# OpenRobotLab/EmbodiedScan

Hardware: AMD Instinct MI355X
Metric: scans/sec (train step) mv-3ddet, 20x(480x640) RGB-D views (higher is better)
Workload: dtype bf16; 1 GPU; mv-3ddet ResNet-50(w16) + MinkResNet34 + FCAF3DHeadRotMat, 20 views 480x640, 100k points/scan, bf16 matrix cores with f32 accumulate / f32 master weights, full train step incl. H2D of the batch and AdamW; views=20, parallelism=dp1, h2d=157 MB per step as ONE copy from a pinned slab on a copy stream, double-buffered

## Files before the change

### embodiedscan_amd/csrc/rowops.hip

```cpp
#include "common.h"
#include "../../include/es_hip.h"

int ES_OPT_NORM_CHUNK = 0;
static int norm_chunk_rows(int max_rows) {
  if (ES_OPT_NORM_CHUNK > 0) return ES_OPT_NORM_CHUNK;
  return max_rows <= (1 << 17) ? 128 : (max_rows <= (1 << 18) ? 256 : 512);
}
#define FCH 16
#define FST 64

struct Segs { int n; int off[ES_MAX_SEG + 1]; };
__device__ inline int seg_of(const Segs& s, int row) {
  int g = 0;
  for (int i = 1; i < s.n; ++i) g += (row >= s.off[i]);
  return g;
}
static Segs make_segs(const int* seg_off, int nseg) {
  Segs s;
  s.n = nseg;
  for (int i = 0; i <= nseg; ++i) s.off[i] = seg_off[i];
  return s;
}
static int max_seg_rows(const Segs& s) {
  int m = 0;
// ... 120 lines not shown
                                                     const float* __restrict__ res, int ldr, int act,
                                                     float* __restrict__ y, int ldy, unsigned short* __restrict__ yh) {
  const int C4 = C >> 2;
  const size_t tot = (size_t)n * C4, stride = (size_t)gridDim.x * blockDim.x;
  for (size_t e0 = (size_t)blockIdx.x * blockDim.x + threadIdx.x; e0 < tot; e0 += 2 * stride) {
    size_t e1 = e0 + stride;
    bool v1 = e1 < tot;
    int r0 = (int)(e0 / C4), c0 = (int)(e0 - (size_t)r0 * C4) * 4;
    int r1 = v1 ? (int)(e1 / C4) : r0, c1 = v1 ? (int)(e1 - (size_t)r1 * C4) * 4 : c0;
    float4 x0 = *(const float4*)(x + (size_t)r0 * ldx + c0), x1 = *(const float4*)(x + (size_t)r1 * ldx + c1);
    float4 q0 = make_float4(0, 0, 0, 0), q1 = q0;
    if (res) { q0 = *(const float4*)(res + (size_t)r0 * ldr + c0); q1 = *(const float4*)(res + (size_t)r1 * ldr + c1); }
#define NA_ONE(xv, qv, r, c)                                                                                   \
    {                                                                                                          \
      int sg = seg_of(segs, r);                                                                                \
      float4 m = *(const float4*)(mean + sg * C + c), is = *(const float4*)(invstd + sg * C + c);             \
      float4 ww = *(const float4*)(w + c), bb = *(const float4*)(b + c);                                       \
      float z0 = (xv.x - m.x) * is.x * ww.x + bb.x, z1 = (xv.y - m.y) * is.y * ww.y + bb.y;                    \
      float z2 = (xv.z - m.z) * is.z * ww.z + bb.z, z3 = (xv.w - m.w) * is.w * ww.w + bb.w;                    \
      if (res) { z0 += qv.x; z1 += qv.y; z2 += qv.z; z3 += qv.w; }                                             \
      z0 = act_fwd(z0, act); z1 = act_fwd(z1, act); z2 = act_fwd(z2, act); z3 = act_fwd(z3, act);             \
      *(float4*)(y + (size_t)r * ldy + c) = make_float4(z0, z1, z2, z3);                                       \
      if (yh) *(uint2*)(yh + (size_t)r * C + c) = make_uint2(es_pack_bf16(z0, z1), es_pack_bf16(z2, z3));      \
    }
    NA_ONE(x0, q0, r0, c0)
    if (v1) NA_ONE(x1, q1, r1, c1)
#undef NA_ONE
  }
}

int ES_OPT_ELECT_SAFE = 0;
int ES_OPT_NORM_CB_ROWS = 4096;
int ES_OPT_NORM_CB_BWD = 1;
#define NCB_TY 128
#define NCB_WAVES 8
__device__ inline void cb_reduce4(double v[4], double (*sm)[4][4]) {
  const int lane = threadIdx.x & 63, wv = threadIdx.x >> 6, tx = threadIdx.x & 3;
#pragma unroll
  for (int i = 0; i < 4; ++i) {
#pragma unroll
    for (int o = 4; o < 64; o <<= 1) v[i] += __shfl_xor(v[i], o, 64);
  }
  __syncthreads();
  if ((lane >> 2) == 0) {
#pragma unroll
    for (int i = 0; i < 4; ++i) sm[wv][tx][i] = v[i];
  }
  __syncthreads();
#pragma unroll
  for (int i = 0; i < 4; ++i) {
    double tot = 0;
#pragma unroll
    for (int w = 0; w < NCB_WAVES; ++w) tot += sm[w][tx][i];
    v[i] = tot;
  }
}
__global__ __launch_bounds__(512) void k_norm_fwd_cb(const float* __restrict__ x, int ldx, int n, int C, float eps,
                                                      const float* __restrict__ w, const float* __restrict__ b,
                                                      const float* __restrict__ res, int ldr, int act, float* running_mean,
                                                      float* running_var, float momentum, float* __restrict__ mean,
                                                      float* __restrict__ invstd, float* __restrict__ y, int ldy,
                                                      unsigned short* __restrict__ yh) {
  __shared__ double sm[NCB_WAVES][4][4];
  const int tx = threadIdx.x & 3, ty = threadIdx.x >> 2, c = blockIdx.x * 16 + tx * 4;
  const float4 k = *(const float4*)(x + c);
  float4 s = make_float4(0, 0, 0, 0), q = make_float4(0, 0, 0, 0);
  for (int rb = ty; rb < n; rb += 4 * NCB_TY) {
    float4 v[4];
#pragma unroll
    for (int u = 0; u < 4; ++u) {
      const int r = rb + u * NCB_TY;
      const float4 t = *(const float4*)(x + (size_t)(r < n ? r : rb) * ldx + c);
      v[u].x = r < n ? t.x : k.x; v[u].y = r < n ? t.y : k.y;
      v[u].z = r < n ? t.z : k.z; v[u].w = r < n ? t.w : k.w;
    }
#pragma unroll
    for (int u = 0; u < 4; ++u) {
      float dx = v[u].x - k.x, dy = v[u].y - k.y, dz = v[u].z - k.z, dw = v[u].w - k.w;
      s.x += dx; s.y += dy; s.z += dz; s.w += dw;
      q.x += dx * dx; q.y += dy * dy; q.z += dz * dz; q.w += dw * dw;
    }
  }
  double a[4] = {s.x, s.y, s.z, s.w}, bq[4] = {q.x, q.y, q.z, q.w};
  cb_reduce4(a, sm);
  cb_reduce4(bq, sm);
  const double inv_n = 1.0 / (double)n;
  const float kk[4] = {k.x, k.y, k.z, k.w};
  float m4[4], is4[4];
#pragma unroll
  for (int i = 0; i < 4; ++i) {
    double ms = a[i] * inv_n, var = bq[i] * inv_n - ms * ms;
    if (var < 0) var = 0;
    m4[i] = (float)((double)kk[i] + ms);
    is4[i] = (float)(1.0 / sqrt(var + (double)eps));
    if (ty == 0) {
      mean[c + i] = m4[i];
      invstd[c + i] = is4[i];
      if (running_mean && n > 1) {
        running_mean[c + i] = (1.f - momentum) * running_mean[c + i] + momentum * m4[i];
        running_var[c + i] = (1.f - momentum) * running_var[c + i] + momentum * (float)(var * n / (n - 1));
      }
    }
  }
  const float4 ww = *(const float4*)(w + c), bb = *(const float4*)(b + c);
  for (int rb = ty; rb < n; rb += 4 * NCB_TY) {
    float4 v[4], qv[4];
#pragma unroll
    for (int u = 0; u < 4; ++u) {
      int r = rb + u * NCB_TY;
      int rc = r < n ? r : rb;
      v[u] = *(const float4*)(x + (size_t)rc * ldx + c);
      if (res) qv[u] = *(const float4*)(res + (size_t)rc * ldr + c);
    }
#pragma unroll
    for (int u = 0; u < 4; ++u) {
      int r = rb + u * NCB_TY;
      if (r >= n) continue;
      float z0 = (v[u].x - m4[0]) * is4[0] * ww.x + bb.x, z1 = (v[u].y - m4[1]) * is4[1] * ww.y + bb.y;
      float z2 = (v[u].z - m4[2]) * is4[2] * ww.z + bb.z, z3 = (v[u].w - m4[3]) * is4[3] * ww.w + bb.w;
      if (res) { z0 += qv[u].x; z1 += qv[u].y; z2 += qv[u].z; z3 += qv[u].w; }
      z0 = act_fwd(z0, act); z1 = act_fwd(z1, act); z2 = act_fwd(z2, act); z3 = act_fwd(z3, act);
      *(float4*)(y + (size_t)r * ldy + c) = make_float4(z0, z1, z2, z3);
      if (yh) *(uint2*)(yh + (size_t)r * C + c) = make_uint2(es_pack_bf16(z0, z1), es_pack_bf16(z2, z3));
    }
  }
}
static bool norm_cb_ok(int n, int C, int nseg) {
  return ES_OPT_NORM_CB_ROWS > 0 && nseg == 1 && n >= 1 && n <= ES_OPT_NORM_CB_ROWS && (C & 15) == 0;
}

extern "C" int es_norm_fwd(const float* x, int ldx, int n, int C, const int* seg_off, int nseg, float eps,
                           const float* weight, const float* bias, const float* res, int ldr, int act,
                           float* running_mean, float* running_var, float momentum, float* mean, float* invstd,
                           float* workspace, float* y, int ldy, void* y_bf16, void* stream) {
  hipStream_t st = (hipStream_t)stream;
  if (n <= 0 || nseg > ES_MAX_SEG) return nseg > ES_MAX_SEG ? -3 : 0;
  Segs s = make_segs(seg_off, nseg);
  const bool vec0 = ((C & 3) == 0) && ((ldx & 3) == 0) && ((ldy & 3) == 0) && (!res || (ldr & 3) == 0) &&
                    (((((uintptr_t)x) | ((uintptr_t)y) | ((uintptr_t)res) | ((uintptr_t)weight) | ((uintptr_t)bias) |
                       ((uintptr_t)mean) | ((uintptr_t)invstd)) & 15) == 0);
  if (vec0 && norm_cb_ok(n, C, nseg) && seg_off[0] == 0 && seg_off[1] == n) {
    hipLaunchKernelGGL(k_norm_fwd_cb, dim3(C / 16), dim3(4 * NCB_TY), 0, st, x, ldx, n, C, eps, weight, bias, res, ldr, act,
                       running_mean, running_var, momentum, mean, invstd, y, ldy, (unsigned short*)y_bf16);
    ES_CHECK_LAUNCH();
    return 0;
  }
  const int NCH = norm_chunk_rows(max_seg_rows(s));
  int nchunk = es_cdiv(max_seg_rows(s), NCH);
  if (nchunk < 1) nchunk = 1;
  hipLaunchKernelGGL(k_norm_stats, dim3(nchunk, nseg), dim3(256), 0, st, x, ldx, C, s, nchunk, NCH,
                     workspace);
  hipLaunchKernelGGL(k_norm_finalize, dim3(es_cdiv(C, FCH), nseg), dim3(FCH * FST), 0, st, workspace, C, s, nchunk, NCH, eps,
                     mean, invstd, running_mean, running_var, momentum);
  const bool vec = ((C & 3) == 0) && ((ldx & 3) == 0) && ((ldy & 3) == 0) && (!res || (ldr & 3) == 0) &&
                   (((((uintptr_t)x) | ((uintptr_t)y) | ((uintptr_t)res) | ((uintptr_t)weight) | ((uintptr_t)bias) |
                      ((uintptr_t)mean) | ((uintptr_t)invstd)) & 15) == 0);
  if (vec) {
    int g = es_cdiv((long long)n * (C >> 2), 512);
    if (g > 8192) g = 8192;
    hipLaunchKernelGGL(k_norm_apply4, dim3(g < 1 ? 1 : g), dim3(256), 0, st, x, ldx, n, C, s, mean, invstd, weight, bias,
                       res, ldr, act, y, ldy, (unsigned short*)y_bf16);
  } else {
    int g = es_cdiv((long long)n * C, 256);
    if (g > 4096) g = 4096;
    hipLaunchKernelGGL(k_norm_apply, dim3(g), dim3(256), 0, st, x, ldx, n, C, s, mean, invstd, weight, bias, res,
                       ldr, act, y, ldy);
    if (y_bf16) return es_cast_rows_bf16(y, ldy, n, C, y_bf16, stream);
  }
  ES_CHECK_LAUNCH();
  return 0;
}
extern "C" size_t es_norm_workspace_floats(int n, int C, const int* seg_off, int nseg) {
  int m = 0;
  for (int i = 0; i < nseg; ++i) m = max(m, seg_off[i + 1] - seg_off[i]);
  int nchunk = es_cdiv(m, norm_chunk_rows(m));
  if (nchunk < 1) nchunk = 1;
// ... 147 lines not shown
                                                         const float* __restrict__ sum_dzx, float* __restrict__ dx,
                                                         int ldo, int accumulate, unsigned short* __restrict__ dxh) {
  const int C4 = C >> 2;
  const size_t tot = (size_t)n * C4, stride = (size_t)gridDim.x * blockDim.x;
  for (size_t e0 = (size_t)blockIdx.x * blockDim.x + threadIdx.x; e0 < tot; e0 += 2 * stride) {
    size_t e1 = e0 + stride;
    bool v1 = e1 < tot;
    int r0 = (int)(e0 / C4), c0 = (int)(e0 - (size_t)r0 * C4) * 4;
    int r1 = v1 ? (int)(e1 / C4) : r0, c1 = v1 ? (int)(e1 - (size_t)r1 * C4) * 4 : c0;
    float4 x0 = *(const float4*)(x + (size_t)r0 * ldx + c0), x1 = *(const float4*)(x + (size_t)r1 * ldx + c1);
    float4 g0 = *(const float4*)(dz + (size_t)r0 * ldd + c0), g1 = *(const float4*)(dz + (size_t)r1 * ldd + c1);
    float4 o0 = make_float4(0, 0, 0, 0), o1 = o0;
    if (accumulate) { o0 = *(const float4*)(dx + (size_t)r0 * ldo + c0); o1 = *(const float4*)(dx + (size_t)r1 * ldo + c1); }
#define NB_ELT(xe, ge, oe, me, ie, we, se, qe) \
    { float xh = ((xe) - (me)) * (ie); float gg = (we) * (ie) * ((ge) - (se) * inv_n - xh * (qe) * inv_n); oe = accumulate ? ((oe) + gg) : gg; }
#define NB_ONE(xv, gv, ov, r, c)                                                                               \
    {                                                                                                          \
      int sg = seg_of(segs, r);                                                                                \
      float inv_n = 1.f / (float)(segs.off[sg + 1] - segs.off[sg]);                                            \
      float4 m = *(const float4*)(mean + sg * C + c), is = *(const float4*)(invstd + sg * C + c);             \
      float4 ww = *(const float4*)(w + c), sd = *(const float4*)(sum_dz + sg * C + c);                         \
      float4 sq = *(const float4*)(sum_dzx + sg * C + c);                                                      \
      NB_ELT(xv.x, gv.x, ov.x, m.x, is.x, ww.x, sd.x, sq.x) NB_ELT(xv.y, gv.y, ov.y, m.y, is.y, ww.y, sd.y, sq.y) \
      NB_ELT(xv.z, gv.z, ov.z, m.z, is.z, ww.z, sd.z, sq.z) NB_ELT(xv.w, gv.w, ov.w, m.w, is.w, ww.w, sd.w, sq.w) \
      *(float4*)(dx + (size_t)r * ldo + c) = ov;                                                               \
      if (dxh) *(uint2*)(dxh + (size_t)r * C + c) = make_uint2(es_pack_bf16(ov.x, ov.y), es_pack_bf16(ov.z, ov.w)); \
    }
    NB_ONE(x0, g0, o0, r0, c0)
    if (v1) NB_ONE(x1, g1, o1, r1, c1)
#undef NB_ONE
#undef NB_ELT
  }
}
__global__ __launch_bounds__(512) void k_norm_bwd_cb(float* __restrict__ dy, int ldd, const float* __restrict__ y, int ldy,
                                                      const float* __restrict__ x, int ldx, int n, int C,
                                                      const float* __restrict__ mean, const float* __restrict__ invstd,
                                                      const float* __restrict__ w, int act, float* dweight, float* dbias,
                                                      float* __restrict__ dx, int ldo, int accumulate,
                                                      unsigned short* __restrict__ dxh) {
  __shared__ double sm[NCB_WAVES][4][4];
  const int tx = threadIdx.x & 3, ty = threadIdx.x >> 2, c = blockIdx.x * 16 + tx * 4;
  const float4 m = *(const float4*)(mean + c), is = *(const float4*)(invstd + c);
  float4 s = make_float4(0, 0, 0, 0), q = make_float4(0, 0, 0, 0);
  for (int rb = ty; rb < n; rb += 4 * NCB_TY) {
    float4 g[4], yv[4], xv[4];
#pragma unroll
    for (int u = 0; u < 4; ++u) {
      int r = rb + u * NCB_TY;
      int rc = r < n ? r : rb;
      g[u] = *(const float4*)(dy + (size_t)rc * ldd + c);
      if (act) yv[u] = *(const float4*)(y + (size_t)rc * ldy + c);
      xv[u] = *(const float4*)(x + (size_t)rc * ldx + c);
    }
#pragma unroll
    for (int u = 0; u < 4; ++u) {
      int r = rb + u * NCB_TY;
      if (r >= n) continue;
      float4 gg = g[u];
      if (act) {
        float4 yy = yv[u];
        if (act == 1) {
          gg.x = yy.x > 0.f ? gg.x : 0.f; gg.y = yy.y > 0.f ? gg.y : 0.f;
          gg.z = yy.z > 0.f ? gg.z : 0.f; gg.w = yy.w > 0.f ? gg.w : 0.f;
        } else {
          gg.x = yy.x > 0.f ? gg.x : gg.x * (yy.x + 1.f); gg.y = yy.y > 0.f ? gg.y : gg.y * (yy.y + 1.f);
          gg.z = yy.z > 0.f ? gg.z : gg.z * (yy.z + 1.f); gg.w = yy.w > 0.f ? gg.w : gg.w * (yy.w + 1.f);
        }
        *(float4*)(dy + (size_t)r * ldd + c) = gg;
      }
      float4 xx = xv[u];
      s.x += gg.x; s.y += gg.y; s.z += gg.z; s.w += gg.w;
      q.x += gg.x * ((xx.x - m.x) * is.x); q.y += gg.y * ((xx.y - m.y) * is.y);
      q.z += gg.z * ((xx.z - m.z) * is.z); q.w += gg.w * ((xx.w - m.w) * is.w);
    }
  }
  double a[4] = {s.x, s.y, s.z, s.w}, bq[4] = {q.x, q.y, q.z, q.w};
  cb_reduce4(a, sm);
  cb_reduce4(bq, sm);
  if (ty == 0) {
#pragma unroll
    for (int i = 0; i < 4; ++i) {
      if (dweight) dweight[c + i] += (float)bq[i];
      if (dbias) dbias[c + i] += (float)a[i];
    }
  }
  const float sd[4] = {(float)a[0], (float)a[1], (float)a[2], (float)a[3]};
  const float sq[4] = {(float)bq[0], (float)bq[1], (float)bq[2], (float)bq[3]};
  const float4 ww = *(const float4*)(w + c);
  const float inv_n = 1.f / (float)n;
  for (int rb = ty; rb < n; rb += 4 * NCB_TY) {
    float4 g[4], xv[4], ov[4];
#pragma unroll
    for (int u = 0; u < 4; ++u) {
      int r = rb + u * NCB_TY;
      int rc = r < n ? r : rb;
      g[u] = *(const float4*)(dy + (size_t)rc * ldd + c);
      xv[u] = *(const float4*)(x + (size_t)rc * ldx + c);
      ov[u] = accumulate ? *(const float4*)(dx + (size_t)rc * ldo + c) : make_float4(0, 0, 0, 0);
    }
#pragma unroll
    for (int u = 0; u < 4; ++u) {
      int r = rb + u * NCB_TY;
      if (r >= n) continue;
#define NCB_ELT(xe, ge, oe, me, ie, we, se, qe) \
      { float xh = ((xe) - (me)) * (ie); float gg = (we) * (ie) * ((ge) - (se) * inv_n - xh * (qe) * inv_n); oe = accumulate ? ((oe) + gg) : gg; }
      NCB_ELT(xv[u].x, g[u].x, ov[u].x, m.x, is.x, ww.x, sd[0], sq[0]) NCB_ELT(xv[u].y, g[u].y, ov[u].y, m.y, is.y, ww.y, sd[1], sq[1])
      NCB_ELT(xv[u].z, g[u].z, ov[u].z, m.z, is.z, ww.z, sd[2], sq[2]) NCB_ELT(xv[u].w, g[u].w, ov[u].w, m.w, is.w, ww.w, sd[3], sq[3])
#undef NCB_ELT
      *(float4*)(dx + (size_t)r * ldo + c) = ov[u];
      if (dxh) *(uint2*)(dxh + (size_t)r * C + c) = make_uint2(es_pack_bf16(ov[u].x, ov[u].y), es_pack_bf16(ov[u].z, ov[u].w));
    }
  }
}
extern "C" int es_norm_bwd(float* dy, int ldd, const float* y, int ldy, const float* x, int ldx, int n, int C,
                           const int* seg_off, int nseg, const float* mean, const float* invstd,
                           const float* weight, int act, float* dweight, float* dbias, float* workspace, float* dx,
                           int ldo, int accumulate, void* dx_bf16, void* stream) {
  hipStream_t st = (hipStream_t)stream;
  if (n <= 0 || nseg > ES_MAX_SEG) return nseg > ES_MAX_SEG ? -3 : 0;
  Segs s = make_segs(seg_off, nseg);
  const int NCH = norm_chunk_rows(max_seg_rows(s));
  int nchunk = es_cdiv(max_seg_rows(s), NCH);
  if (nchunk < 1) nchunk = 1;
  {
    const bool vec0 = ((C & 3) == 0) && ((ldx & 3) == 0) && ((ldd & 3) == 0) && ((ldo & 3) == 0) && ((ldy & 3) == 0) &&
                      (((((uintptr_t)x) | ((uintptr_t)dy) | ((uintptr_t)dx) | ((uintptr_t)y) | ((uintptr_t)weight) |
                         ((uintptr_t)mean) | ((uintptr_t)invstd)) & 15) == 0);
    if (vec0 && dx != dy && ES_OPT_NORM_CB_BWD && norm_cb_ok(n, C, nseg) && seg_off[0] == 0 && seg_off[1] == n) {
      hipLaunchKernelGGL(k_norm_bwd_cb, dim3(C / 16), dim3(4 * NCB_TY), 0, st, dy, ldd, y, ldy, x, ldx, n, C, mean, invstd, weight, act,
                         dweight, dbias, dx, ldo, accumulate, (unsigned short*)dx_bf16);
      ES_CHECK_LAUNCH();
      return 0;
    }
  }
  float* sums = workspace + (size_t)nseg * nchunk * 2 * C;
  hipLaunchKernelGGL(k_norm_bwd_stats, dim3(nchunk, nseg), dim3(256), 0, st, dy, ldd, y, ldy, x,
                     ldx, C, s, nchunk, NCH, mean, invstd, act, workspace);
  hipLaunchKernelGGL(k_norm_bwd_finalize, dim3(es_cdiv(C, FCH)), dim3(FCH * FST), 0, st, workspace, C, s, nchunk, NCH, sums,
                     sums + (size_t)nseg * C, dweight, dbias);
  const bool vec = ((C & 3) == 0) && ((ldx & 3) == 0) && ((ldd & 3) == 0) && ((ldo & 3) == 0) &&
                   (((((uintptr_t)x) | ((uintptr_t)dy) | ((uintptr_t)dx) | ((uintptr_t)weight) | ((uintptr_t)mean) |
                      ((uintptr_t)invstd) | ((uintptr_t)sums)) & 15) == 0) && ((((size_t)nseg * C) & 3) == 0);
  if (vec && dx != dy) {
    int g = es_cdiv((long long)n * (C >> 2), 512);
    if (g > 8192) g = 8192;
    hipLaunchKernelGGL(k_norm_bwd_apply4, dim3(g < 1 ? 1 : g), dim3(256), 0, st, dy, ldd, x, ldx, n, C, s, mean, invstd,
                       weight, sums, sums + (size_t)nseg * C, dx, ldo, accumulate, (unsigned short*)dx_bf16);
  } else {
    int g = es_cdiv((long long)n * C, 256);
    if (g > 4096) g = 4096;
    hipLaunchKernelGGL(k_norm_bwd_apply, dim3(g), dim3(256), 0, st, dy, ldd, x, ldx, n, C, s, mean, invstd, weight,
                       sums, sums + (size_t)nseg * C, dx, ldo, accumulate);
    if (dx_bf16) return es_cast_rows_bf16(dx, ldo, n, C, dx_bf16, stream);
  }
  ES_CHECK_LAUNCH();
  return 0;
}

__global__ void k_maxpool_fwd(const float* __restrict__ x, int ldx, const int* __restrict__ nbr, int n_out, int K,
                              int C, float* __restrict__ y, int* __restrict__ arg) {
  size_t tot = (size_t)n_out * C;
  for (size_t e = (size_t)blockIdx.x * blockDim.x + threadIdx.x; e < tot; e += (size_t)gridDim.x * blockDim.x) {
    int j = (int)(e / C), c = (int)(e - (size_t)j * C);
// ... 579 lines not shown
```

### embodiedscan_amd/csrc/spconv.hip

```cpp
#include "common.h"
#include "../../include/es_hip.h"

typedef float f32x4 __attribute__((ext_vector_type(4)));

static int ES_OPT_PINGPONG = 1;
static int ES_OPT_WGRAD_HUGE = 1;
static int ES_OPT_ROWGEMM = 1;
static int ES_OPT_WG_BIG_TARGET = 2048;
static int ES_OPT_WG_BIG_ROWS = 512;
static int ES_OPT_WG_SMALL_TARGET = 1024;
static int ES_OPT_WG_CAP_MB = 256;
static int ES_OPT_FWD_SPLIT_WGS = 384;
static int ES_OPT_DMA = 2;
static int ES_OPT_DMA_MIN_CIN = 768;
static int ES_OPT_WGRAD_TR = 1;
static int ES_OPT_ROWGEMM2 = 1;
static int ES_OPT_SPLIT_FOLD = 0;
static int ES_OPT_RG128_MIN_CIN = 0;
static int ES_OPT_NARROW_SLICES = 768;
static int ES_OPT_LIN_SMALL = 256;
static int ES_OPT_EXPAND = 65536;
static int ES_OPT_EXPAND_WGS = 1024;
static int ES_OPT_RG320 = 1;
static int ES_OPT_NARROW = 1;
static int ES_OPT_WSHARE = 0;
static int ES_OPT_RG128_MIN_WGS = 0;
extern int ES_OPT_NORM_CB_ROWS;
extern int ES_OPT_NORM_CB_BWD;
extern int ES_OPT_ELECT_SAFE;
extern int ES_OPT_NORM_CHUNK;
extern "C" int es_set_option(int key, int value) {
  if (key == 1) { ES_OPT_PINGPONG = value; return 0; }
  if (key == 2) { ES_OPT_WGRAD_HUGE = value; return 0; }
  if (key == 3) { ES_OPT_ROWGEMM = value; return 0; }
  if (key == 4) { ES_OPT_WG_BIG_TARGET = value; return 0; }
  if (key == 5) { ES_OPT_WG_BIG_ROWS = value; return 0; }
  if (key == 6) { ES_OPT_WG_SMALL_TARGET = value; return 0; }
  if (key == 7) { ES_OPT_WG_CAP_MB = value; return 0; }
  if (key == 8) { ES_OPT_FWD_SPLIT_WGS = value; return 0; }
  if (key == 9) { ES_OPT_NORM_CHUNK = value; return 0; }
  if (key == 10) { ES_OPT_DMA = value; return 0; }
  if (key == 11) { ES_OPT_DMA_MIN_CIN = value; return 0; }
  if (key == 12) { ES_OPT_RG128_MIN_CIN = value; return 0; }
  if (key == 13) { ES_OPT_ROWGEMM2 = value; return 0; }
  if (key == 14) { ES_OPT_WGRAD_TR = value; return 0; }
  if (key == 15) { ES_OPT_NORM_CB_ROWS = value; return 0; }
  if (key == 16) { ES_OPT_SPLIT_FOLD = value; return 0; }
  if (key == 17) { ES_OPT_NORM_CB_BWD = value; return 0; }
  if (key == 18) { ES_OPT_ELECT_SAFE = value; return 0; }
  if (key == 19) { ES_OPT_RG128_MIN_WGS = value; return 0; }
  if (key == 20) { ES_OPT_WSHARE = value; return 0; }
  if (key == 21) { ES_OPT_NARROW = value; return 0; }
  if (key == 22) { ES_OPT_NARROW_SLICES = value; return 0; }
  if (key == 23) { ES_OPT_RG320 = value; return 0; }
  if (key == 24) { ES_OPT_LIN_SMALL = value; return 0; }
  if (key == 25) { ES_OPT_EXPAND = value; return 0; }
  if (key == 26) { ES_OPT_EXPAND_WGS = value; return 0; }
  return -2;
}


#define BM 128
#define BN 64
#define BK 16
#define LDB (BN + 16)
#define MAXK 27

__device__ inline int a_swz(int row_k) { return (((row_k >> 2) & 3) << 3) ^ ((row_k & 1) << 4); }

template <bool TRANS_W>
__global__ __launch_bounds__(256) void k_spconv(const float* __restrict__ X, int ldx, const float* __restrict__ W,
                                                const int* __restrict__ nbr, int n_out, int n_in, int K, int Cin,
                                                int Cout, const float* __restrict__ bias, float* __restrict__ Y,
                                                int ldy, int accumulate) {
  __shared__ float As[BK * BM];
  __shared__ float Bs[BK * LDB];
  __shared__ int nbrS[BM * MAXK];
  __shared__ int tapAny[32];

  const int t = threadIdx.x, lane = t & 63, wv = t >> 6;
  const int row0 = blockIdx.x * BM, n0 = blockIdx.y * BN;
  const bool vecA = ((ldx & 3) == 0) && ((((uintptr_t)X) & 15) == 0);
  const bool vecB = TRANS_W ? (((Cin & 3) == 0) && ((((uintptr_t)W) & 15) == 0))
                            : (((Cout & 3) == 0) && ((((uintptr_t)W) & 15) == 0));

  if (t < 32) tapAny[t] = 0;
  __syncthreads();
  for (int e = t; e < BM * K; e += 256) {
    int r = e / K, k = e - r * K;
    int j = row0 + r, v = -1;
// ... 2706 lines not shown
```

### embodiedscan_amd/hip.py

```python
import ctypes
import os
import re

_HERE = os.path.dirname(os.path.abspath(__file__))
LIB_PATH = os.path.join(_HERE, 'libes_hip.so')
HEADER_PATH = os.path.join(os.path.dirname(_HERE), 'include', 'es_hip.h')

_CT = {'int': ctypes.c_int, 'float': ctypes.c_float, 'double': ctypes.c_double, 'size_t': ctypes.c_size_t}


def parse_header(path=HEADER_PATH):
    src = open(path).read()
    src = re.sub(r'/\*.*?\*/', ' ', src, flags=re.S)
    out = {}
    for m in re.finditer(r'\b(int|size_t)\s+(es_\w+)\s*\(([^)]*)\)\s*;', src):
        ret, name, args = m.group(1), m.group(2), m.group(3)
        at, an = [], []
        for a in args.split(','):
            a = a.strip()
            if not a or a == 'void':
                continue
            an.append(re.findall(r'(\w+)\s*$', a)[0])
            if '*' in a:
                at.append(ctypes.c_void_p)
            else:
                toks = [t for t in a.split() if t != 'const']
                at.append(_CT[toks[0]])
        out[name] = (_CT[ret], at, an)
    return out


PROTOS = parse_header()
CONSTS = {k: int(v) for k, v in re.findall(r'#define\s+(ES_\w+)\s+(\d+)', open(HEADER_PATH).read())}

if not os.path.exists(LIB_PATH):
    raise ImportError(f'{LIB_PATH} is missing: build it with `make -C embodiedscan_amd/csrc` '
                      '(or __graft_entry__.build()); there is no CPU fallback for the HIP path')
_lib = ctypes.CDLL(LIB_PATH)
_fn = {}
for _name, (_ret, _at, _an) in PROTOS.items():
    _f = getattr(_lib, _name)
    _f.restype, _f.argtypes = _ret, _at
    _fn[_name] = _f


if os.environ.get('ES_PINGPONG') is not None:
    _fn['es_set_option'](1, int(os.environ['ES_PINGPONG']))
if os.environ.get('ES_WGRAD_HUGE') is not None:
    _fn['es_set_option'](2, int(os.environ['ES_WGRAD_HUGE']))
if os.environ.get('ES_ROWGEMM') is not None:
    _fn['es_set_option'](3, int(os.environ['ES_ROWGEMM']))
for _key, _env in ((4, 'ES_WG_BIG_TARGET'), (5, 'ES_WG_BIG_ROWS'), (6, 'ES_WG_SMALL_TARGET'), (7, 'ES_WG_CAP_MB'), (8, 'ES_FWD_SPLIT_WGS'),
                  (10, 'ES_DMA'), (11, 'ES_DMA_MIN_CIN'), (12, 'ES_RG128_MIN_CIN'), (14, 'ES_WGRAD_TR'), (15, 'ES_NORM_CB_ROWS'),
                  (16, 'ES_SPLIT_FOLD'), (19, 'ES_RG128_MIN_WGS'), (20, 'ES_WSHARE'), (21, 'ES_NARROW'), (23, 'ES_RG320'), (24, 'ES_LIN_SMALL'), (25, 'ES_EXPAND'), (26, 'ES_EXPAND_WGS')):
    if os.environ.get(_env) is not None:
        _fn['es_set_option'](_key, int(os.environ[_env]))


class HipError(RuntimeError):
    pass


PROFILE = None
PAIRS = {}


def register_map(nbr):
    if PROFILE is not None and nbr is not None:
        PAIRS[nbr.data_ptr()] = (nbr >= 0).sum()
    return nbr


_EXT_STREAMS = {}


def _stream_of(handle):
    import torch
    st = _EXT_STREAMS.get(handle)
    if st is None:
        st = _EXT_STREAMS[handle] = torch.cuda.ExternalStream(handle) if handle else torch.cuda.default_stream()
    return st


def _launch(name, args):
    prof = PROFILE
    if prof is not None and name in prof['names']:
        e0, e1 = prof['event'](), prof['event']()
# ... 66 lines not shown
```

### include/es_hip.h

```cpp
#ifndef ES_HIP_H
#define ES_HIP_H
#include <stddef.h>
#include <stdint.h>
#ifdef __cplusplus
extern "C" {
#endif

#define ES_MAX_SEG 32

#define ES_MAX_BATCH 512
int es_voxel_keys(const float* points, int n, int ld, int batch, float voxel_size, int64_t* keys, void* stream);
int es_unique_first(const int64_t* keys, int n, int64_t* tkeys, int* tvals, int cap, int* scratch,
                    int64_t* out_keys, int* out_src, int* count_host, void* stream);
size_t es_sort_scratch_bytes(int n);
int es_morton_sort(const int64_t* keys, const int* src, int n, void* scratch, size_t scratch_bytes, int64_t* out_keys,
                   int* out_src, void* stream);
int es_sort_u64(const int64_t* keys, const int* src, int n, void* scratch, size_t scratch_bytes, int64_t* out_keys, int* out_src,
                void* stream);
int es_draw_keys(const float* depth, int V, int HW, size_t seed, float* values, int64_t* keys, void* stream);
int es_draw_keys_index(int n, size_t seed, int stream_id, float* values, int64_t* keys, void* stream);
int es_draw_unpack(const int64_t* keys, int n, const int* in_view, const int* in_pix, int* out_view, int* out_pix, void* stream);
int es_build_table(const int64_t* keys, int n, int64_t* tkeys, int* tvals, int cap, void* stream);
int es_stride_keys(const int64_t* in_keys, int n, int out_ts, int64_t* out_keys, void* stream);
int es_keys_to_coords(const int64_t* keys, int n, int* coords , void* stream);
// ... 21 lines not shown
size_t es_spconv_split_workspace_floats(int n_out, int K, int Cin, int Cout);
int es_spconv_fwd_bf16_ws(const void* X, int x_is_bf16, int ldx, const void* W_bf16, const int* nbr, int n_out, int n_in,
                          int K, int Cin, int Cout, const float* bias, float* Y, int ldy, int accumulate, float* ws,
                          size_t ws_floats, void* stream);
int es_spconv_bf16_is_fast(int n_in, int ldx, int K, int Cin, int Cout);
int es_gen_transpose_fwd_bf16(const float* X, int ldx, const void* Wt_bf16, int n, int Cin, int Cout, float* Y, void* stream);
int es_gen_transpose_dgrad_bf16(const float* dY, const void* Wn_bf16, int n, int Cin, int Cout, float* dX, int ldx,
                                int accumulate, void* stream);
int es_gen_transpose_wgrad_bf16(const float* X, int ldx, const float* dY , int n, int Cin, int Cout,
                                float* dW , int accumulate, float* ws, size_t ws_floats, void* stream);
size_t es_gen_transpose_wgrad_workspace_floats(const float* X, int ldx, const float* dY, int n, int Cin, int Cout);
int es_set_option(int key, int value);
int es_spconv_fwd_bf16_affine(const void* X, int ldx, const void* W_bf16, const int* nbr, int n_out, int n_in, int K,
                              int Cin, int Cout, const float* scale, const float* shift, const float* res, int ldr,
                              int act, float* Y, int ldy, void* stream);
int es_spconv_fwd_bf16_io(const void* X, int x_half, int ldx, const void* W_bf16, const int* nbr, int n_out, int n_in, int K,
                          int Cin, int Cout, const float* scale, const float* shift, const void* res, int res_half, int ldr,
                          int act, void* Y, int y_half, int ldy, void* stream);
int es_cast_rows_bf16(const float* x, int ldx, int n, int C, void* h , void* stream);
int es_cast_weight_bf16(const float* w, int K, int A, int B, void* natural, void* transposed, void* stream);
int es_cast_weights_table(const void* table_dev, int n_entries, int total_tiles, void* stream);
int es_spconv_wgrad(const float* X, int ldx, const float* dY, int ldy, const int* nbr, int n_out, int n_in, int K,
                    int Cin, int Cout, float* dW, int accumulate, float* ws, size_t ws_floats, void* stream);
int es_spconv_wgrad_bf16(const float* X, int ldx, const float* dY, int ldy, const int* nbr, int n_out, int n_in, int K,
                         int Cin, int Cout, float* dW, int accumulate, float* ws, size_t ws_floats, void* stream);
int es_spconv_wgrad_bf16_src(const void* X, int x_half, int ldx, const void* dY, int dy_half, int ldy, const int* nbr,
                             int n_out, int n_in, int K, int Cin, int Cout, float* dW, int accumulate, float* ws,
                             size_t ws_floats, void* stream);
size_t es_spconv_wgrad_workspace_floats(int bf16, const void* X, int x_half, int ldx, const void* dY, int dy_half, int ldy,
                                        int n_out, int n_in, int K, int Cin, int Cout);
int es_image_map(int n_img, int H, int W, int Ho, int Wo, int KH, int KW, int stride, int pad, int* nbr, void* stream);

size_t es_norm_workspace_floats(int n, int C, const int* seg_off_host, int nseg);
int es_norm_fwd(const float* x, int ldx, int n, int C, const int* seg_off_host, int nseg, float eps,
                const float* weight, const float* bias, const float* res, int ldr, int act, float* running_mean,
                float* running_var, float momentum, float* mean, float* invstd, float* workspace, float* y, int ldy,
                void* y_bf16, void* stream);
int es_norm_bwd(float* dy, int ldd, const float* y, int ldy, const float* x, int ldx, int n, int C,
                const int* seg_off_host, int nseg, const float* mean, const float* invstd, const float* weight,
                int act, float* dweight, float* dbias, float* workspace, float* dx, int ldo, int accumulate,
                void* dx_bf16, void* stream);
int es_maxpool_fwd(const float* x, int ldx, const int* nbr, int n_out, int K, int C, float* y, int* arg, void* stream);
int es_maxpool_fwd_h(const float* x, int ldx, const int* nbr, int n_out, int K, int C, void* y_bf16, void* stream);
int es_maxpool_bwd(const float* dy, const int* arg, int n_out, int C, float* dx, int ldo, void* stream);
int es_row_move(float* dst, int ldd, const float* src, int lds, const int* idx, int n, int C, int mode, void* stream);
int es_axpy2d(float* dst, int ldd, const float* src, int lds, int n, int C, float alpha, int op, void* stream);
int es_interp_scores(const float* score, const int* idx, const float* w, int n, float* out, void* stream);
size_t es_colsum_workspace_floats(int n, int C);
int es_colsum(const float* g, int ld, int n, int C, float* dst, int accumulate, float* workspace, size_t workspace_floats, void* stream);
int es_topk_mask(const float* values, const int* seg_off_host, int nseg, int k, int* mask, void* stream);
size_t es_topk_mask_workspace_ints(int nseg);
int es_topk_mask_ws(const float* values, const int* seg_off_host, int nseg, int k, int* mask, int* workspace, size_t workspace_ints,
                    void* stream);
int es_row_max(const float* x, int ldx, int n, int C, float* out, void* stream);
int es_bn_fold(const float* w, const float* b, const float* rm, const float* rv, int C, float eps, float* scale,
               float* shift, void* stream);
int es_affine_act_fwd(const float* x, const float* scale, const float* shift, const float* res, size_t n, int C,
                      int act, float* y, void* stream);
int es_affine_act_bwd(const float* dy, const float* y, const float* scale, size_t n, int C, int act, float* dx,
                      int acc_x, float* dres, int acc_r, void* stream);
int es_affine_act_bwd_yh(const float* dy, const void* y_bf16, const float* scale, size_t n, int C, int act, float* dx,
                         int acc_x, float* dres, int acc_r, void* stream);

#define ES_FUSE_NOPS 0
#define ES_FUSE_OPS 1
#define ES_FUSE_ROTINV 9
// ... 207 lines not shown
```

Before: 180.5 scans/s.

## Cache column-block norm rows in registers and adapt channels per block

The column-block batch-norm forward and backward kernels now load up to 8 row tiles per thread into registers once. Both the statistics pass and the apply pass reuse them, so small inputs no longer read x (and dy/res) from memory twice. The number of channels per workgroup now drops from 16 to 8 or 4 as rows grow, which launches more workgroups for small-row layers. The two reductions are merged into one with a single barrier, and block indices are swizzled. The trade-off is higher register pressure (up to 32 float4 arrays in backward), which may reduce occupancy.

```diff
diff --git a/embodiedscan_amd/csrc/rowops.hip b/embodiedscan_amd/csrc/rowops.hip
--- a/embodiedscan_amd/csrc/rowops.hip
+++ b/embodiedscan_amd/csrc/rowops.hip
@@ -176,64 +176,86 @@
 int ES_OPT_ELECT_SAFE = 0;
 int ES_OPT_NORM_CB_ROWS = 4096;
 int ES_OPT_NORM_CB_BWD = 1;
-#define NCB_TY 128
+int ES_OPT_NORM_CB_CH = 0;
+#define NCB_THREADS 512
 #define NCB_WAVES 8
-__device__ inline void cb_reduce4(double v[4], double (*sm)[4][4]) {
-  const int lane = threadIdx.x & 63, wv = threadIdx.x >> 6, tx = threadIdx.x & 3;
-#pragma unroll
-  for (int i = 0; i < 4; ++i) {
-#pragma unroll
-    for (int o = 4; o < 64; o <<= 1) v[i] += __shfl_xor(v[i], o, 64);
+#define NCB_R 8
+#define NCB_LOADS_DONE() __builtin_amdgcn_s_waitcnt(0x0F70)
+static int norm_cb_channels(int n, int C) {
+  if (ES_OPT_NORM_CB_CH == 16 || ES_OPT_NORM_CB_CH == 8 || ES_OPT_NORM_CB_CH == 4) return ES_OPT_NORM_CB_CH;
+  (void)C;
+  return n <= 128 * NCB_R ? 16 : (n <= 256 * NCB_R ? 8 : 4);
+}
+extern "C" int es_norm_cb_channels(int n, int C) { return norm_cb_channels(n, C); }
+__device__ inline int cb_block() {
+  const int g = blockIdx.x, G = gridDim.x;
+  return (G & 7) == 0 ? (g & 7) * (G >> 3) + (g >> 3) : g;
+}
+template <int TXN>
+__device__ inline void cb_reduce8(double v[8], double (*sm)[4][8]) {
+  const int lane = threadIdx.x & 63, wv = threadIdx.x >> 6, tx = threadIdx.x & (TXN - 1);
+#pragma unroll
+  for (int i = 0; i < 8; ++i) {
+#pragma unroll
+    for (int o = TXN; o < 64; o <<= 1) v[i] += __shfl_xor(v[i], o, 64);
+  }
+  if (lane < TXN) {
+#pragma unroll
+    for (int i = 0; i < 8; ++i) sm[wv][tx][i] = v[i];
   }
   __syncthreads();
-  if ((lane >> 2) == 0) {
-#pragma unroll
-    for (int i = 0; i < 4; ++i) sm[wv][tx][i] = v[i];
-  }
-  __syncthreads();
-#pragma unroll
-  for (int i = 0; i < 4; ++i) {
+#pragma unroll
+  for (int i = 0; i < 8; ++i) {
     double tot = 0;
 #pragma unroll
     for (int w = 0; w < NCB_WAVES; ++w) tot += sm[w][tx][i];
     v[i] = tot;
   }
 }
-__global__ __launch_bounds__(512) void k_norm_fwd_cb(const float* __restrict__ x, int ldx, int n, int C, float eps,
-                                                      const float* __restrict__ w, const float* __restrict__ b,
-                                                      const float* __restrict__ res, int ldr, int act, float* running_mean,
-                                                      float* running_var, float momentum, float* __restrict__ mean,
-                                                      float* __restrict__ invstd, float* __restrict__ y, int ldy,
-                                                      unsigned short* __restrict__ yh) {
-  __shared__ double sm[NCB_WAVES][4][4];
-  const int tx = threadIdx.x & 3, ty = threadIdx.x >> 2, c = blockIdx.x * 16 + tx * 4;
+template <int CPW>
+__device__ __forceinline__ void norm_fwd_cb(const float* __restrict__ x, int ldx, int n, int C, float eps,
+                                            const float* __restrict__ w, const float* __restrict__ b,
+                                            const float* __restrict__ res, int ldr, int act, float* running_mean,
+                                            float* running_var, float momentum, float* __restrict__ mean,
+                                            float* __restrict__ invstd, float* __restrict__ y, int ldy,
+                                            unsigned short* __restrict__ yh, double (*sm)[4][8]) {
+  constexpr int TXN = CPW / 4, L = NCB_THREADS / TXN;
+  const int tx = threadIdx.x & (TXN - 1), ty = threadIdx.x / TXN, c = cb_block() * CPW + tx * 4;
   const float4 k = *(const float4*)(x + c);
+  float4 xv[NCB_R], qv[NCB_R];
+#pragma unroll
+  for (int u = 0; u < NCB_R; ++u) {
+    if (u * L < n) {
+      const int r = ty + u * L, rc = r < n ? r : 0;
+      xv[u] = *(const float4*)(x + (size_t)rc * ldx + c);
+      if (res) qv[u] = *(const float4*)(res + (size_t)rc * ldr + c);
+    }
+  }
+  const float4 ww = *(const float4*)(w + c), bb = *(const float4*)(b + c);
+  NCB_LOADS_DONE();
   float4 s = make_float4(0, 0, 0, 0), q = make_float4(0, 0, 0, 0);
-  for (int rb = ty; rb < n; rb += 4 * NCB_TY) {
-    float4 v[4];
-#pragma unroll
-    for (int u = 0; u < 4; ++u) {
-      const int r = rb + u * NCB_TY;
-      const float4 t = *(const float4*)(x + (size_t)(r < n ? r : rb) * ldx + c);
-      v[u].x = r < n ? t.x : k.x; v[u].y = r < n ? t.y : k.y;
-      v[u].z = r < n ? t.z : k.z; v[u].w = r < n ? t.w : k.w;
-    }
-#pragma unroll
-    for (int u = 0; u < 4; ++u) {
-      float dx = v[u].x - k.x, dy = v[u].y - k.y, dz = v[u].z - k.z, dw = v[u].w - k.w;
-      s.x += dx; s.y += dy; s.z += dz; s.w += dw;
-      q.x += dx * dx; q.y += dy * dy; q.z += dz * dz; q.w += dw * dw;
-    }
-  }
-  double a[4] = {s.x, s.y, s.z, s.w}, bq[4] = {q.x, q.y, q.z, q.w};
-  cb_reduce4(a, sm);
-  cb_reduce4(bq, sm);
+#define NCB_STAT(v)                                                                       \
+  {                                                                                       \
+    float dx = (v).x - k.x, dy = (v).y - k.y, dz = (v).z - k.z, dw = (v).w - k.w;         \
+    s.x += dx; s.y += dy; s.z += dz; s.w += dw;                                           \
+    q.x += dx * dx; q.y += dy * dy; q.z += dz * dz; q.w += dw * dw;                       \
+  }
+#pragma unroll
+  for (int u = 0; u < NCB_R; ++u)
+    if (ty + u * L < n) NCB_STAT(xv[u])
+  for (int r = ty + NCB_R * L; r < n; r += L) {
+    const float4 t = *(const float4*)(x + (size_t)r * ldx + c);
+    NCB_STAT(t)
+  }
+#undef NCB_STAT
+  double a[8] = {s.x, s.y, s.z, s.w, q.x, q.y, q.z, q.w};
+  cb_reduce8<TXN>(a, sm);
   const double inv_n = 1.0 / (double)n;
   const float kk[4] = {k.x, k.y, k.z, k.w};
   float m4[4], is4[4];
 #pragma unroll
   for (int i = 0; i < 4; ++i) {
-    double ms = a[i] * inv_n, var = bq[i] * inv_n - ms * ms;
+    double ms = a[i] * inv_n, var = a[4 + i] * inv_n - ms * ms;
     if (var < 0) var = 0;
     m4[i] = (float)((double)kk[i] + ms);
     is4[i] = (float)(1.0 / sqrt(var + (double)eps));
@@ -246,28 +268,36 @@
       }
     }
   }
-  const float4 ww = *(const float4*)(w + c), bb = *(const float4*)(b + c);
-  for (int rb = ty; rb < n; rb += 4 * NCB_TY) {
-    float4 v[4], qv[4];
-#pragma unroll
-    for (int u = 0; u < 4; ++u) {
-      int r = rb + u * NCB_TY;
-      int rc = r < n ? r : rb;
-      v[u] = *(const float4*)(x + (size_t)rc * ldx + c);
-      if (res) qv[u] = *(const float4*)(res + (size_t)rc * ldr + c);
-    }
-#pragma unroll
-    for (int u = 0; u < 4; ++u) {
-      int r = rb + u * NCB_TY;
-      if (r >= n) continue;
-      float z0 = (v[u].x - m4[0]) * is4[0] * ww.x + bb.x, z1 = (v[u].y - m4[1]) * is4[1] * ww.y + bb.y;
-      float z2 = (v[u].z - m4[2]) * is4[2] * ww.z + bb.z, z3 = (v[u].w - m4[3]) * is4[3] * ww.w + bb.w;
-      if (res) { z0 += qv[u].x; z1 += qv[u].y; z2 += qv[u].z; z3 += qv[u].w; }
-      z0 = act_fwd(z0, act); z1 = act_fwd(z1, act); z2 = act_fwd(z2, act); z3 = act_fwd(z3, act);
-      *(float4*)(y + (size_t)r * ldy + c) = make_float4(z0, z1, z2, z3);
-      if (yh) *(uint2*)(yh + (size_t)r * C + c) = make_uint2(es_pack_bf16(z0, z1), es_pack_bf16(z2, z3));
-    }
-  }
+#define NCB_APPLY(v, qq, r)                                                                                    \
+  {                                                                                                            \
+    float z0 = ((v).x - m4[0]) * is4[0] * ww.x + bb.x, z1 = ((v).y - m4[1]) * is4[1] * ww.y + bb.y;            \
+    float z2 = ((v).z - m4[2]) * is4[2] * ww.z + bb.z, z3 = ((v).w - m4[3]) * is4[3] * ww.w + bb.w;            \
+    if (res) { z0 += (qq).x; z1 += (qq).y; z2 += (qq).z; z3 += (qq).w; }                                       \
+    z0 = act_fwd(z0, act); z1 = act_fwd(z1, act); z2 = act_fwd(z2, act); z3 = act_fwd(z3, act);               \
+    *(float4*)(y + (size_t)(r) * ldy + c) = make_float4(z0, z1, z2, z3);                                       \
+    if (yh) *(uint2*)(yh + (size_t)(r) * C + c) = make_uint2(es_pack_bf16(z0, z1), es_pack_bf16(z2, z3));      \
+  }
+#pragma unroll
+  for (int u = 0; u < NCB_R; ++u)
+    if (ty + u * L < n) NCB_APPLY(xv[u], qv[u], ty + u * L)
+  for (int r = ty + NCB_R * L; r < n; r += L) {
+    const float4 t = *(const float4*)(x + (size_t)r * ldx + c);
+    float4 tq = make_float4(0, 0, 0, 0);
+    if (res) tq = *(const float4*)(res + (size_t)r * ldr + c);
+    NCB_APPLY(t, tq, r)
+  }
+#undef NCB_APPLY
+}
+__global__ __launch_bounds__(NCB_THREADS) void k_norm_fwd_cb(const float* __restrict__ x, int ldx, int n, int C, float eps,
+                                                              const float* __restrict__ w, const float* __restrict__ b,
+                                                              const float* __restrict__ res, int ldr, int act, float* running_mean,
+                                                              float* running_var, float momentum, float* __restrict__ mean,
+                                                              float* __restrict__ invstd, float* __restrict__ y, int ldy,
+                                                              unsigned short* __restrict__ yh, int cpw) {
+  __shared__ double sm[NCB_WAVES][4][8];
+  if (cpw == 16) norm_fwd_cb<16>(x, ldx, n, C, eps, w, b, res, ldr, act, running_mean, running_var, momentum, mean, invstd, y, ldy, yh, sm);
+  else if (cpw == 8) norm_fwd_cb<8>(x, ldx, n, C, eps, w, b, res, ldr, act, running_mean, running_var, momentum, mean, invstd, y, ldy, yh, sm);
+  else norm_fwd_cb<4>(x, ldx, n, C, eps, w, b, res, ldr, act, running_mean, running_var, momentum, mean, invstd, y, ldy, yh, sm);
 }
 static bool norm_cb_ok(int n, int C, int nseg) {
   return ES_OPT_NORM_CB_ROWS > 0 && nseg == 1 && n >= 1 && n <= ES_OPT_NORM_CB_ROWS && (C & 15) == 0;
@@ -284,8 +314,9 @@
                     (((((uintptr_t)x) | ((uintptr_t)y) | ((uintptr_t)res) | ((uintptr_t)weight) | ((uintptr_t)bias) |
                        ((uintptr_t)mean) | ((uintptr_t)invstd)) & 15) == 0);
   if (vec0 && norm_cb_ok(n, C, nseg) && seg_off[0] == 0 && seg_off[1] == n) {
-    hipLaunchKernelGGL(k_norm_fwd_cb, dim3(C / 16), dim3(4 * NCB_TY), 0, st, x, ldx, n, C, eps, weight, bias, res, ldr, act,
-                       running_mean, running_var, momentum, mean, invstd, y, ldy, (unsigned short*)y_bf16);
+    const int cpw = norm_cb_channels(n, C);
+    hipLaunchKernelGGL(k_norm_fwd_cb, dim3(C / cpw), dim3(NCB_THREADS), 0, st, x, ldx, n, C, eps, weight, bias, res, ldr, act,
+                       running_mean, running_var, momentum, mean, invstd, y, ldy, (unsigned short*)y_bf16, cpw);
     ES_CHECK_LAUNCH();
     return 0;
   }
@@ -499,85 +530,99 @@
 #undef NB_ELT
   }
 }
-__global__ __launch_bounds__(512) void k_norm_bwd_cb(float* __restrict__ dy, int ldd, const float* __restrict__ y, int ldy,
-                                                      const float* __restrict__ x, int ldx, int n, int C,
-                                                      const float* __restrict__ mean, const float* __restrict__ invstd,
-                                                      const float* __restrict__ w, int act, float* dweight, float* dbias,
-                                                      float* __restrict__ dx, int ldo, int accumulate,
-                                                      unsigned short* __restrict__ dxh) {
-  __shared__ double sm[NCB_WAVES][4][4];
-  const int tx = threadIdx.x & 3, ty = threadIdx.x >> 2, c = blockIdx.x * 16 + tx * 4;
-  const float4 m = *(const float4*)(mean + c), is = *(const float4*)(invstd + c);
-  float4 s = make_float4(0, 0, 0, 0), q = make_float4(0, 0, 0, 0);
-  for (int rb = ty; rb < n; rb += 4 * NCB_TY) {
-    float4 g[4], yv[4], xv[4];
-#pragma unroll
-    for (int u = 0; u < 4; ++u) {
-      int r = rb + u * NCB_TY;
-      int rc = r < n ? r : rb;
+template <int CPW>
+__device__ __forceinline__ void norm_bwd_cb(float* __restrict__ dy, int ldd, const float* __restrict__ y, int ldy,
+                                            const float* __restrict__ x, int ldx, int n, int C,
+                                            const float* __restrict__ mean, const float* __restrict__ invstd,
+                                            const float* __restrict__ w, int act, float* dweight, float* dbias,
+                                            float* __restrict__ dx, int ldo, int accumulate,
+                                            unsigned short* __restrict__ dxh, double (*sm)[4][8]) {
+  constexpr int TXN = CPW / 4, L = NCB_THREADS / TXN;
+  const int tx = threadIdx.x & (TXN - 1), ty = threadIdx.x / TXN, c = cb_block() * CPW + tx * 4;
+  const float4 m = *(const float4*)(mean + c), is = *(const float4*)(invstd + c), ww = *(const float4*)(w + c);
+  float4 g[NCB_R], yv[NCB_R], xv[NCB_R], ov[NCB_R];
+#pragma unroll
+  for (int u = 0; u < NCB_R; ++u) {
+    if (u * L < n) {
+      const int r = ty + u * L, rc = r < n ? r : 0;
       g[u] = *(const float4*)(dy + (size_t)rc * ldd + c);
       if (act) yv[u] = *(const float4*)(y + (size_t)rc * ldy + c);
       xv[u] = *(const float4*)(x + (size_t)rc * ldx + c);
-    }
-#pragma unroll
-    for (int u = 0; u < 4; ++u) {
-      int r = rb + u * NCB_TY;
-      if (r >= n) continue;
-      float4 gg = g[u];
-      if (act) {
-        float4 yy = yv[u];
-        if (act == 1) {
-          gg.x = yy.x > 0.f ? gg.x : 0.f; gg.y = yy.y > 0.f ? gg.y : 0.f;
-          gg.z = yy.z > 0.f ? gg.z : 0.f; gg.w = yy.w > 0.f ? gg.w : 0.f;
-        } else {
-          gg.x = yy.x > 0.f ? gg.x : gg.x * (yy.x + 1.f); gg.y = yy.y > 0.f ? gg.y : gg.y * (yy.y + 1.f);
-          gg.z = yy.z > 0.f ? gg.z : gg.z * (yy.z + 1.f); gg.w = yy.w > 0.f ? gg.w : gg.w * (yy.w + 1.f);
-        }
-        *(float4*)(dy + (size_t)r * ldd + c) = gg;
-      }
-      float4 xx = xv[u];
-      s.x += gg.x; s.y += gg.y; s.z += gg.z; s.w += gg.w;
-      q.x += gg.x * ((xx.x - m.x) * is.x); q.y += gg.y * ((xx.y - m.y) * is.y);
-      q.z += gg.z * ((xx.z - m.z) * is.z); q.w += gg.w * ((xx.w - m.w) * is.w);
-    }
-  }
-  double a[4] = {s.x, s.y, s.z, s.w}, bq[4] = {q.x, q.y, q.z, q.w};
-  cb_reduce4(a, sm);
-  cb_reduce4(bq, sm);
+      if (accumulate) ov[u] = *(const float4*)(dx + (size_t)rc * ldo + c);
+    }
+  }
+  NCB_LOADS_DONE();
+  float4 s = make_float4(0, 0, 0, 0), q = make_float4(0, 0, 0, 0);
+#define NCB_GATE(gg, yy, xx, r)                                                                                \
+  {                                                                                                            \
+    if (act) {                                                                                                 \
+      if (act == 1) {                                                                                          \
+        (gg).x = (yy).x > 0.f ? (gg).x : 0.f; (gg).y = (yy).y > 0.f ? (gg).y : 0.f;                            \
+        (gg).z = (yy).z > 0.f ? (gg).z : 0.f; (gg).w = (yy).w > 0.f ? (gg).w : 0.f;                            \
+      } else {                                                                                                 \
+        (gg).x = (yy).x > 0.f ? (gg).x : (gg).x * ((yy).x + 1.f); (gg).y = (yy).y > 0.f ? (gg).y : (gg).y * ((yy).y + 1.f); \
+        (gg).z = (yy).z > 0.f ? (gg).z : (gg).z * ((yy).z + 1.f); (gg).w = (yy).w > 0.f ? (gg).w : (gg).w * ((yy).w + 1.f); \
+      }                                                                                                        \
+      *(float4*)(dy + (size_t)(r) * ldd + c) = (gg);                                                           \
+    }                                                                                                          \
+    s.x += (gg).x; s.y += (gg).y; s.z += (gg).z; s.w += (gg).w;                                                \
+    q.x += (gg).x * (((xx).x - m.x) * is.x); q.y += (gg).y * (((xx).y - m.y) * is.y);                          \
+    q.z += (gg).z * (((xx).z - m.z) * is.z); q.w += (gg).w * (((xx).w - m.w) * is.w);                          \
+  }
+#pragma unroll
+  for (int u = 0; u < NCB_R; ++u)
+    if (ty + u * L < n) NCB_GATE(g[u], yv[u], xv[u], ty + u * L)
+  for (int r = ty + NCB_R * L; r < n; r += L) {
+    float4 tg = *(const float4*)(dy + (size_t)r * ldd + c), tyv = make_float4(0, 0, 0, 0);
+    if (act) tyv = *(const float4*)(y + (size_t)r * ldy + c);
+    const float4 tx4 = *(const float4*)(x + (size_t)r * ldx + c);
+    NCB_GATE(tg, tyv, tx4, r)
+  }
+#undef NCB_GATE
+  double a[8] = {s.x, s.y, s.z, s.w, q.x, q.y, q.z, q.w};
+  cb_reduce8<TXN>(a, sm);
   if (ty == 0) {
 #pragma unroll
     for (int i = 0; i < 4; ++i) {
-      if (dweight) dweight[c + i] += (float)bq[i];
+      if (dweight) dweight[c + i] += (float)a[4 + i];
       if (dbias) dbias[c + i] += (float)a[i];
     }
   }
   const float sd[4] = {(float)a[0], (float)a[1], (float)a[2], (float)a[3]};
-  const float sq[4] = {(float)bq[0], (float)bq[1], (float)bq[2], (float)bq[3]};
-  const float4 ww = *(const float4*)(w + c);
+  const float sq[4] = {(float)a[4], (float)a[5], (float)a[6], (float)a[7]};
   const float inv_n = 1.f / (float)n;
-  for (int rb = ty; rb < n; rb += 4 * NCB_TY) {
-    float4 g[4], xv[4], ov[4];
-#pragma unroll
-    for (int u = 0; u < 4; ++u) {
-      int r = rb + u * NCB_TY;
-      int rc = r < n ? r : rb;
-      g[u] = *(const float4*)(dy + (size_t)rc * ldd + c);
-      xv[u] = *(const float4*)(x + (size_t)rc * ldx + c);
-      ov[u] = accumulate ? *(const float4*)(dx + (size_t)rc * ldo + c) : make_float4(0, 0, 0, 0);
-    }
-#pragma unroll
-    for (int u = 0; u < 4; ++u) {
-      int r = rb + u * NCB_TY;
-      if (r >= n) continue;
 #define NCB_ELT(xe, ge, oe, me, ie, we, se, qe) \
-      { float xh = ((xe) - (me)) * (ie); float gg = (we) * (ie) * ((ge) - (se) * inv_n - xh * (qe) * inv_n); oe = accumulate ? ((oe) + gg) : gg; }
-      NCB_ELT(xv[u].x, g[u].x, ov[u].x, m.x, is.x, ww.x, sd[0], sq[0]) NCB_ELT(xv[u].y, g[u].y, ov[u].y, m.y, is.y, ww.y, sd[1], sq[1])
-      NCB_ELT(xv[u].z, g[u].z, ov[u].z, m.z, is.z, ww.z, sd[2], sq[2]) NCB_ELT(xv[u].w, g[u].w, ov[u].w, m.w, is.w, ww.w, sd[3], sq[3])
+  { float xh = ((xe) - (me)) * (ie); float gg = (we) * (ie) * ((ge) - (se) * inv_n - xh * (qe) * inv_n); oe = accumulate ? ((oe) + gg) : gg; }
+#define NCB_APPLY(xx, gg, oo, r)                                                                                                   \
+  {                                                                                                                                \
+    NCB_ELT((xx).x, (gg).x, (oo).x, m.x, is.x, ww.x, sd[0], sq[0]) NCB_ELT((xx).y, (gg).y, (oo).y, m.y, is.y, ww.y, sd[1], sq[1]) \
+    NCB_ELT((xx).z, (gg).z, (oo).z, m.z, is.z, ww.z, sd[2], sq[2]) NCB_ELT((xx).w, (gg).w, (oo).w, m.w, is.w, ww.w, sd[3], sq[3]) \
+    *(float4*)(dx + (size_t)(r) * ldo + c) = (oo);                                                                                 \
+    if (dxh) *(uint2*)(dxh + (size_t)(r) * C + c) = make_uint2(es_pack_bf16((oo).x, (oo).y), es_pack_bf16((oo).z, (oo).w));        \
+  }
+#pragma unroll
+  for (int u = 0; u < NCB_R; ++u)
+    if (ty + u * L < n) NCB_APPLY(xv[u], g[u], ov[u], ty + u * L)
+  for (int r = ty + NCB_R * L; r < n; r += L) {
+    const float4 tg = *(const float4*)(dy + (size_t)r * ldd + c);
+    const float4 tx4 = *(const float4*)(x + (size_t)r * ldx + c);
+    float4 to = make_float4(0, 0, 0, 0);
+    if (accumulate) to = *(const float4*)(dx + (size_t)r * ldo + c);
+    NCB_APPLY(tx4, tg, to, r)
+  }
+#undef NCB_APPLY
 #undef NCB_ELT
-      *(float4*)(dx + (size_t)r * ldo + c) = ov[u];
-      if (dxh) *(uint2*)(dxh + (size_t)r * C + c) = make_uint2(es_pack_bf16(ov[u].x, ov[u].y), es_pack_bf16(ov[u].z, ov[u].w));
-    }
-  }
+}
+__global__ __launch_bounds__(NCB_THREADS) void k_norm_bwd_cb(float* __restrict__ dy, int ldd, const float* __restrict__ y, int ldy,
+                                                              const float* __restrict__ x, int ldx, int n, int C,
+                                                              const float* __restrict__ mean, const float* __restrict__ invstd,
+                                                              const float* __restrict__ w, int act, float* dweight, float* dbias,
+                                                              float* __restrict__ dx, int ldo, int accumulate,
+                                                              unsigned short* __restrict__ dxh, int cpw) {
+  __shared__ double sm[NCB_WAVES][4][8];
+  if (cpw == 16) norm_bwd_cb<16>(dy, ldd, y, ldy, x, ldx, n, C, mean, invstd, w, act, dweight, dbias, dx, ldo, accumulate, dxh, sm);
+  else if (cpw == 8) norm_bwd_cb<8>(dy, ldd, y, ldy, x, ldx, n, C, mean, invstd, w, act, dweight, dbias, dx, ldo, accumulate, dxh, sm);
+  else norm_bwd_cb<4>(dy, ldd, y, ldy, x, ldx, n, C, mean, invstd, w, act, dweight, dbias, dx, ldo, accumulate, dxh, sm);
 }
 extern "C" int es_norm_bwd(float* dy, int ldd, const float* y, int ldy, const float* x, int ldx, int n, int C,
                            const int* seg_off, int nseg, const float* mean, const float* invstd,
@@ -594,8 +639,9 @@
                       (((((uintptr_t)x) | ((uintptr_t)dy) | ((uintptr_t)dx) | ((uintptr_t)y) | ((uintptr_t)weight) |
                          ((uintptr_t)mean) | ((uintptr_t)invstd)) & 15) == 0);
     if (vec0 && dx != dy && ES_OPT_NORM_CB_BWD && norm_cb_ok(n, C, nseg) && seg_off[0] == 0 && seg_off[1] == n) {
-      hipLaunchKernelGGL(k_norm_bwd_cb, dim3(C / 16), dim3(4 * NCB_TY), 0, st, dy, ldd, y, ldy, x, ldx, n, C, mean, invstd, weight, act,
-                         dweight, dbias, dx, ldo, accumulate, (unsigned short*)dx_bf16);
+      const int cpw = norm_cb_channels(n, C);
+      hipLaunchKernelGGL(k_norm_bwd_cb, dim3(C / cpw), dim3(NCB_THREADS), 0, st, dy, ldd, y, ldy, x, ldx, n, C, mean, invstd, weight, act,
+                         dweight, dbias, dx, ldo, accumulate, (unsigned short*)dx_bf16, cpw);
       ES_CHECK_LAUNCH();
       return 0;
     }
diff --git a/embodiedscan_amd/csrc/spconv.hip b/embodiedscan_amd/csrc/spconv.hip
--- a/embodiedscan_amd/csrc/spconv.hip
+++ b/embodiedscan_amd/csrc/spconv.hip
@@ -27,6 +27,7 @@
 static int ES_OPT_RG128_MIN_WGS = 0;
 extern int ES_OPT_NORM_CB_ROWS;
 extern int ES_OPT_NORM_CB_BWD;
+extern int ES_OPT_NORM_CB_CH;
 extern int ES_OPT_ELECT_SAFE;
 extern int ES_OPT_NORM_CHUNK;
 extern "C" int es_set_option(int key, int value) {
@@ -56,6 +57,7 @@
   if (key == 24) { ES_OPT_LIN_SMALL = value; return 0; }
   if (key == 25) { ES_OPT_EXPAND = value; return 0; }
   if (key == 26) { ES_OPT_EXPAND_WGS = value; return 0; }
+  if (key == 27) { ES_OPT_NORM_CB_CH = value; return 0; }
   return -2;
 }
 
diff --git a/embodiedscan_amd/hip.py b/embodiedscan_amd/hip.py
--- a/embodiedscan_amd/hip.py
+++ b/embodiedscan_amd/hip.py
@@ -52,7 +52,8 @@
     _fn['es_set_option'](3, int(os.environ['ES_ROWGEMM']))
 for _key, _env in ((4, 'ES_WG_BIG_TARGET'), (5, 'ES_WG_BIG_ROWS'), (6, 'ES_WG_SMALL_TARGET'), (7, 'ES_WG_CAP_MB'), (8, 'ES_FWD_SPLIT_WGS'),
                   (10, 'ES_DMA'), (11, 'ES_DMA_MIN_CIN'), (12, 'ES_RG128_MIN_CIN'), (14, 'ES_WGRAD_TR'), (15, 'ES_NORM_CB_ROWS'),
-                  (16, 'ES_SPLIT_FOLD'), (19, 'ES_RG128_MIN_WGS'), (20, 'ES_WSHARE'), (21, 'ES_NARROW'), (23, 'ES_RG320'), (24, 'ES_LIN_SMALL'), (25, 'ES_EXPAND'), (26, 'ES_EXPAND_WGS')):
+                  (16, 'ES_SPLIT_FOLD'), (19, 'ES_RG128_MIN_WGS'), (20, 'ES_WSHARE'), (21, 'ES_NARROW'), (23, 'ES_RG320'), (24, 'ES_LIN_SMALL'), (25, 'ES_EXPAND'), (26, 'ES_EXPAND_WGS'),
+                  (27, 'ES_NORM_CB_CH')):
     if os.environ.get(_env) is not None:
         _fn['es_set_option'](_key, int(os.environ[_env]))
 
diff --git a/include/es_hip.h b/include/es_hip.h
--- a/include/es_hip.h
+++ b/include/es_hip.h
@@ -77,6 +77,7 @@
 int es_image_map(int n_img, int H, int W, int Ho, int Wo, int KH, int KW, int stride, int pad, int* nbr, void* stream);
 
 size_t es_norm_workspace_floats(int n, int C, const int* seg_off_host, int nseg);
+int es_norm_cb_channels(int n, int C);
 int es_norm_fwd(const float* x, int ldx, int n, int C, const int* seg_off_host, int nseg, float eps,
                 const float* weight, const float* bias, const float* res, int ldr, int act, float* running_mean,
                 float* running_var, float momentum, float* mean, float* invstd, float* workspace, float* y, int ldy,
```

After: 182.2 scans/s, median of 6. No clear change (+1.0%).
